# JiapengWu/TeMP

Hardware: AMD Instinct MI355X
Metric: edges/sec (fwd+bwd) RGCN+GRU seq_len=15 (higher is better)
Workload: dtype f32

## Files before the change

### temp_amd/csrc/common.hpp

```cpp
#pragma once
#include <hip/hip_runtime.h>
#include <stdint.h>
#include <stddef.h>
#include "temp_amd.h"

#define TEMP_WAVE 64

namespace temp {

typedef float f32x4 __attribute__((ext_vector_type(4)));
typedef float f32x16 __attribute__((ext_vector_type(16)));

__device__ __forceinline__ float4 ld4(const float* p) { return *reinterpret_cast<const float4*>(p); }
__device__ __forceinline__ void st4(float* p, float4 v) { *reinterpret_cast<float4*>(p) = v; }
__device__ __forceinline__ float4 ld4_nt(const float* p) {
  const f32x4 v = __builtin_nontemporal_load(reinterpret_cast<const f32x4*>(p));
  return make_float4(v[0], v[1], v[2], v[3]);
}
__device__ __forceinline__ void st4_nt(float* p, float4 v) {
  f32x4 x = {v.x, v.y, v.z, v.w};
  __builtin_nontemporal_store(x, reinterpret_cast<f32x4*>(p));
}
__device__ __forceinline__ float4 zero4() { return make_float4(0.f, 0.f, 0.f, 0.f); }
__device__ __forceinline__ float4 add4(float4 a, float4 b) { return make_float4(a.x + b.x, a.y + b.y, a.z + b.z, a.w + b.w); }
// ... 54 lines not shown
  r.end = c_hi;
  r.stride = bpx * per_block;
  return r;
}

struct DropSpec { float p; float inv_keep; unsigned long long seed; };
inline DropSpec drop_spec(const TempDropout* d) {
  DropSpec s{0.f, 1.f, 0ull};
  if (d && d->p > 0.f) { s.p = d->p; s.inv_keep = 1.f / (1.f - d->p); s.seed = d->seed; }
  return s;
}
__device__ __forceinline__ float drop_scale(const DropSpec& d, unsigned row, unsigned col) {
  unsigned long long x = d.seed ^ (((unsigned long long)row << 32) | col);
  x ^= x >> 33; x *= 0xff51afd7ed558ccdULL; x ^= x >> 33; x *= 0xc4ceb9fe1a85ec53ULL; x ^= x >> 33;
  const float u = (float)(x >> 40) * (1.0f / 16777216.0f);
  return u < d.p ? 0.f : d.inv_keep;
}
__device__ __forceinline__ float4 drop4(const DropSpec& d, unsigned row, unsigned col, float4 v) {
  return make_float4(v.x * drop_scale(d, row, col), v.y * drop_scale(d, row, col + 1), v.z * drop_scale(d, row, col + 2),
                     v.w * drop_scale(d, row, col + 3));
}

int option(int key);
void hx_count();

inline int ceil_div(long long a, long long b) { return (int)((a + b - 1) / b); }
inline size_t align_up(size_t x, size_t a) { return (x + a - 1) / a * a; }

enum KernelId {
  K_RGCN_AGG_FWD = 0, K_RGCN_AGG_DX, K_RGCN_DW, K_FIXUP, K_GEMM_LOOP_FWD, K_GEMM_LOOP_DX, K_GEMM_TN, K_REDUCE_SLICES, K_COLSUM,
  K_RELU_BWD, K_GRU_FWD, K_GRU_BWD_GATES, K_GEMM_GRU_DX, K_GEMM_GRU_DPREV, K_GATHER_ROWS, K_SCATTER_ADD, K_DECAY_GRAD, K_COPY,
  K_GEMM_ISO, K_GEMM_GRU_GI, K_GEMM_LINEAR, K_GATHER_CE, K_SA_ATTN_FWD, K_SA_ATTN_BWD, K_GRU_CHAIN_FWD, K_GRU_CHAIN_BWD,
  K_GRU_CHAIN_PACK, K_BX_PACK, K_GEMM_TN_BX8, K_GEMM_TN_BX, K_GRU_WGRAD, K_SEGMENT_SUM, K_KEYS, K_GATED_QUERY, K_GATHER_CE_MIX,
  K_PAIR_MSG, K_PAIR_GATHER_FWD, K_PAIR_FIX_EPI, K_PAIR_GATHER_BWD, K_PAIR_DTABLE, K_PAIR_DW, K_COUNT
};
int trace_open(int kernel_id, hipStream_t st);
void trace_close(int slot, hipStream_t st);
#define TEMP_LAUNCH(KID, kernel, grid, block, shmem, st, ...)            \
  do {                                                                   \
    const int _slot = ::temp::trace_open((KID), (st));                   \
    hipLaunchKernelGGL(kernel, grid, block, shmem, st, __VA_ARGS__);     \
    ::temp::trace_close(_slot, (st));                                    \
  } while (0)

inline int launch_status() {
  hipError_t e = hipGetLastError();
  return e == hipSuccess ? TEMP_OK : TEMP_E_LAUNCH;
}

struct EpiAddBiasAct;

int gemm_add_bias_act(int kid, int M, int N, int K, const float* A, int lda, const int32_t* a_idx,
                      const float* B, int ldb, int trans_b,
                      const float* addend, int ld_add, const int32_t* row_mask, const float* bias, int act,
                      float* out, int ldo, hipStream_t st, const DropSpec* drop = nullptr);

int gemm_bias_multi(int kid, int count, const int* Ms, int N, int K, const float* const* As, const int32_t* const* a_idxs , int lda,
                    const float* const* Bs, int ldb,
                    const float* const* biases, float* const* outs, int ldo, hipStream_t st,
                    const unsigned* const* a_keys = nullptr );

int mask_rows(int n, int d, const float* src, float* dst, const DropSpec& drop, hipStream_t st);

size_t gemm_tn_workspace(int M, int Ka, int Nb);
bool gemm_tn_can_fuse_bias(int Nb);
int gemm_tn(int M, int Ka, int Nb, const float* A, int lda, const float* B, int ldb,
            float* out, int ldo, void* ws, size_t ws_bytes, hipStream_t st, float* bias_out = nullptr);
// ... 21 lines not shown
```

### temp_amd/csrc/gemm_kernels.hip

```cpp
#include "common.hpp"
#include <type_traits>
#include <mutex>
#include <atomic>
#include <cstdlib>
#include "gemm_wres.hpp"
#include "gemm_tn_bx.hpp"

namespace temp {

struct EpiAddBiasAct {
  const float* addend; int ld_add; const int32_t* row_mask; const float* bias; int act; float* out; int ldo;
  struct RowCtx { int add; };
  __device__ __forceinline__ RowCtx row_ctx(int row) const {
    RowCtx c;
    c.add = !addend ? 0 : (row_mask ? row_mask[row] : 1);
    return c;
  }
  __device__ __forceinline__ float4 pre4(const RowCtx& c, int row, int col) const {
    float4 a = zero4();
    if (addend) {
      const float4 v = ld4(addend + (size_t)row * ld_add + col);
      a = c.add > 0 ? v : zero4();
    }
    if (bias) a = add4(a, ld4(bias + col));
// ... 1022 lines not shown
  g_options[TEMP_OPT_GEMM_STREAM] = 0; g_options[TEMP_OPT_GRU_STREAM] = 0; g_options[TEMP_OPT_RGCN_TILE] = 1; g_options[TEMP_OPT_DEBUG] = 0; g_options[TEMP_OPT_OVERLAP] = 1; g_options[TEMP_OPT_GEMM_RESIDENT] = 1;
  g_options[TEMP_OPT_MFMA_F16X2] = 1;
  g_options[TEMP_OPT_RGCN_PAIR] = 1;
  const char* e;
  if ((e = getenv("TEMP_MFMA")) && e[0] == 'f' && e[1] == '3') g_options[TEMP_OPT_MFMA_BF16X3] = 0;
  if ((e = getenv("TEMP_MFMA")) && e[0] == 'b') g_options[TEMP_OPT_MFMA_F16X2] = 0;
  if ((e = getenv("TEMP_TN_SPLIT")) && e[0] == '0') g_options[TEMP_OPT_TN_SPLIT] = 0;
  if ((e = getenv("TEMP_RGCN_SCALAR")) && e[0] == '0') g_options[TEMP_OPT_RGCN_SCALAR] = 0;
  if ((e = getenv("TEMP_GEMM_STREAM")) && e[0] == '1') g_options[TEMP_OPT_GEMM_STREAM] = 1;
  if ((e = getenv("TEMP_GRU_STREAM")) && e[0] == '1') g_options[TEMP_OPT_GRU_STREAM] = 1;
  if ((e = getenv("TEMP_RGCN_TILE")) && e[0] >= '0' && e[0] <= '9') g_options[TEMP_OPT_RGCN_TILE] = atoi(e);
  if ((e = getenv("TEMP_OVERLAP")) && e[0] == '0') g_options[TEMP_OPT_OVERLAP] = 0;
  if ((e = getenv("TEMP_GEMM_RESIDENT")) && e[0] == '0') g_options[TEMP_OPT_GEMM_RESIDENT] = 0;
  if ((e = getenv("TEMP_DEBUG"))) g_options[TEMP_OPT_DEBUG] = atoi(e);
  if ((e = getenv("TEMP_RGCN_PAIR")) && e[0] >= '0' && e[0] <= '9') g_options[TEMP_OPT_RGCN_PAIR] = atoi(e);
  return true;
}();
int option(int key) { return (key >= 0 && key < TEMP_OPT_COUNT) ? g_options[key].load(std::memory_order_relaxed) : -1; }
static std::atomic<long long> g_hx_launches{0};
void hx_count() { g_hx_launches.fetch_add(1, std::memory_order_relaxed); }
long long hx_launches() { return g_hx_launches.load(std::memory_order_relaxed); }
}

extern "C" {

const char* temp_trace_kernel_name(int id) {
  static const char* names[] = {"k_rgcn_agg<fwd>", "k_rgcn_agg<dx>", "k_rgcn_dw", "k_fixup", "k_gemm_panel<loop_fwd>",
                                "k_gemm_panel<loop_dx>", "k_gemm_tn", "k_reduce_slices", "k_colsum_part", "k_relu_bwd", "k_gru_fwd",
                                "k_gru_bwd_gates", "k_gemm_panel<gru_dx>", "k_gemm_panel<gru_dprev>", "k_gather_rows",
                                "k_scatter_add_rows", "k_decay_grad", "k_copy", "k_gemm_panel<isolated>", "k_gemm_panel<gru_gi>",
                                "k_gemm_panel<linear>", "k_gather_ce", "k_sa_attn_fwd", "k_sa_attn_bwd", "k_gru_chain_fwd", "k_gru_chain_bwd",
                                "k_gru_chain_pack", "k_bx_pack", "k_gemm_tn_bx8", "k_gemm_tn_bx", "k_gru_wgrad", "k_segment_sum_rows", "k_absmax_keys",
                                "k_gated_query", "k_gather_ce_mix", "k_pair_msg", "k_pair_gather<fwd>", "k_pair_fix_epi", "k_pair_gather<bwd>",
                                "k_pair_dtable", "k_pair_dw"};
  static_assert(sizeof(names) / sizeof(names[0]) == K_COUNT, "one name per KernelId");
  return (id >= 0 && id < K_COUNT) ? names[id] : "?";
}

int temp_abi_version(void) { return TEMP_ABI_VERSION; }

int temp_set_option(int key, int value) {
  if (key < 0 || key >= TEMP_OPT_COUNT) return -1;
  return temp::g_options[key].exchange(value, std::memory_order_relaxed);
}
int temp_get_option(int key) { return temp::option(key); }
long long temp_scratch_refused(void) { return temp::bx_scratch_refused(); }
long long temp_f16_launches(void) { return temp::hx_launches(); }

const char* temp_error_string(int code) {
  switch (code) {
    case TEMP_OK: return "ok";
    case TEMP_E_BADARG: return "bad argument (NULL, negative or inconsistent)";
    case TEMP_E_UNSUPPORTED: return "shape not supported by the gfx950 kernels";
    case TEMP_E_WORKSPACE: return "workspace missing or too small";
    case TEMP_E_LAUNCH: return "HIP launch failure";
    default: return "unknown error";
  }
}

int temp_rgcn_isolated_fwd(int n, int d, const float* e, const float* loop_w, const float* bias, int act, float* out, const TempDropout* drop,
                           void* stream) {
  if (n < 0 || d <= 0 || !loop_w || (n > 0 && (!e || !out))) return TEMP_E_BADARG;
  if (d % 4) return TEMP_E_UNSUPPORTED;
  const DropSpec ds = drop_spec(drop);
  return gemm_add_bias_act(K_GEMM_ISO, n, d, d, e, d, nullptr, loop_w, d, 0, e, d, nullptr, bias, act, out, d, (hipStream_t)stream, &ds);
}

// ... 650 lines not shown
```

### temp_amd/csrc/rgcn_kernels.hip

```cpp
#include <stdlib.h>
#include <atomic>
#include <mutex>
#include "common.hpp"
#include "side_stream.hpp"

namespace temp {

enum { MODE_FWD = 0, MODE_DX = 1 };

template <int S, int MODE>
__device__ __forceinline__ void block_mac(float4& acc, const float4 x, const float4* w, const float c) {
  if (S == 1) {
    acc.x = fmaf(c * x.x, w[0].x, acc.x);
    acc.y = fmaf(c * x.y, w[0].y, acc.y);
    acc.z = fmaf(c * x.z, w[0].z, acc.z);
    acc.w = fmaf(c * x.w, w[0].w, acc.w);
  } else if (S == 2) {
    const float x0 = c * x.x, x1 = c * x.y, x2 = c * x.z, x3 = c * x.w;
    if (MODE == MODE_FWD) {
      acc.x = fmaf(x0, w[0].x, fmaf(x1, w[0].z, acc.x));
      acc.y = fmaf(x0, w[0].y, fmaf(x1, w[0].w, acc.y));
      acc.z = fmaf(x2, w[1].x, fmaf(x3, w[1].z, acc.z));
      acc.w = fmaf(x2, w[1].y, fmaf(x3, w[1].w, acc.w));
    } else {
// ... 834 lines not shown
      };
      int e = 0;
      for (; e + 8 <= cnt; e += 8) {
        float4 x[8];
#pragma unroll
        for (int u = 0; u < 8; ++u) x[u] = row(e + u);
#pragma unroll
        for (int u = 0; u < 8; ++u) add(e + u, x[u]);
      }
      for (; e + 2 <= cnt; e += 2) {
        const float4 x0 = row(e), x1 = row(e + 1);
        add(e, x0);
        add(e + 1, x1);
      }
      if (e < cnt) add(e, row(e));
    }
  }
  return acc;
}

__device__ __forceinline__ float4 pair_epilogue(float4 v, int node, int f, int D, const int32_t* __restrict__ ids, const float* __restrict__ t_loop,
                                                const float* __restrict__ bias, int act, const DropSpec& drop) {
  float4 lm = ld4(t_loop + (size_t)ids[node] * D + f);
  if (drop.p > 0.f) lm = drop4(drop, (unsigned)node, (unsigned)f, lm);
  v = add4(v, lm);
  if (bias) v = add4(v, ld4(bias + f));
  if (act == TEMP_ACT_RELU) v = make_float4(fmaxf(v.x, 0.f), fmaxf(v.y, 0.f), fmaxf(v.z, 0.f), fmaxf(v.w, 0.f));
  return v;
}

__global__ void __launch_bounds__(256) k_pair_gather_fwd(TempEdgeView v, const int32_t* __restrict__ fwd_row, const float* __restrict__ M,
                                                         const float* __restrict__ nnorm, int D, const int32_t* __restrict__ ids,
                                                         const float* __restrict__ t_loop, const float* __restrict__ bias, int act, DropSpec drop,
                                                         float* __restrict__ out, float* __restrict__ partial) {
  const int lane = threadIdx.x & 63;
  const int wave = __builtin_amdgcn_readfirstlane(threadIdx.x >> 6), wpb = blockDim.x >> 6;
  const int f = lane << 2;
  const bool active = lane < (D >> 2);
  ItemRange it = xcd_chunks(v.n_chunks, v.n_edges, v.chunk_beg, wpb);
  for (int c = it.beg + wave; c < it.end; c += it.stride) {
    const int seg = __builtin_amdgcn_readfirstlane(v.chunk_seg[c]), beg = __builtin_amdgcn_readfirstlane(v.chunk_beg[c]);
    const int end = __builtin_amdgcn_readfirstlane(v.chunk_end[c]), slot = __builtin_amdgcn_readfirstlane(v.chunk_slot[c]);
    float4 acc = pair_rows_sum<false>(fwd_row, beg, end, M, D, nullptr, lane, active);
    if (!active) continue;
    const float nn = nnorm[seg];
    acc = scale4(acc, nn * nn);
    if (slot < 0) st4(out + (size_t)seg * D + f, pair_epilogue(acc, seg, f, D, ids, t_loop, bias, act, drop));
    else st4(partial + (size_t)slot * D + f, acc);
  }
}

__global__ void __launch_bounds__(256) k_pair_fix_epi(int n_fix, const int32_t* __restrict__ fix_seg, const int32_t* __restrict__ fix_slot,
                                                      const int32_t* __restrict__ fix_cnt, const float* __restrict__ partial, int n_nodes,
                                                      const int32_t* __restrict__ in_deg, int D, const int32_t* __restrict__ ids,
                                                      const float* __restrict__ t_loop, const float* __restrict__ bias, int act, DropSpec drop,
                                                      float* __restrict__ out) {
  const int lane = threadIdx.x & 63, wpb = blockDim.x >> 6;
  const int gw = blockIdx.x * wpb + (threadIdx.x >> 6), waves = gridDim.x * wpb;
  const int f = lane << 2;
  if (f >= D) return;
  for (int i = gw; i < n_fix; i += waves) {
    const int seg = fix_seg[i];
    st4(out + (size_t)seg * D + f, pair_epilogue(fixup_walk(partial + (size_t)fix_slot[i] * D + f, 0, fix_cnt[i], D), seg, f, D, ids, t_loop, bias, act, drop));
  }
  for (int node = gw; node < n_nodes; node += waves)
    if (in_deg[node] <= 0) st4(out + (size_t)node * D + f, pair_epilogue(zero4(), node, f, D, ids, t_loop, bias, act, drop));
}

__global__ void __launch_bounds__(256) k_pair_gather_bwd(TempEdgeView v, const float* __restrict__ dz, const float* __restrict__ nnorm, int D,
                                                         float* __restrict__ G, float* __restrict__ partial) {
  const int lane = threadIdx.x & 63;
  const int wave = __builtin_amdgcn_readfirstlane(threadIdx.x >> 6), wpb = blockDim.x >> 6;
  const int f = lane << 2;
  const bool active = lane < (D >> 2);
  for (int c = blockIdx.x * wpb + wave; c < v.n_chunks; c += gridDim.x * wpb) {
    const int seg = __builtin_amdgcn_readfirstlane(v.chunk_seg[c]), beg = __builtin_amdgcn_readfirstlane(v.chunk_beg[c]);
    const int end = __builtin_amdgcn_readfirstlane(v.chunk_end[c]), slot = __builtin_amdgcn_readfirstlane(v.chunk_slot[c]);
    const float4 acc = pair_rows_sum<true>(v.a, beg, end, dz, D, nnorm, lane, active);
    if (active) st4((slot < 0 ? G + (size_t)seg * D : partial + (size_t)slot * D) + f, acc);
  }
}

template <int S>
__global__ void __launch_bounds__(64) k_pair_dtable(int n_table, int n_rel_rows, int D, const float* __restrict__ G, const float* __restrict__ W,
                                                    float* __restrict__ d_table) {
  const int D4 = D >> 2;
  const int i = blockIdx.x * blockDim.x + threadIdx.x;
  if (i >= n_table * D4) return;
  const int e = i / D4, f = (i - e * D4) << 2;
  float4 acc = zero4();
#pragma unroll 4
  for (int r = 0; r < n_rel_rows; ++r) {
    const float* wr = W + (size_t)r * (D * S) + f * S;
    float4 w[S];
#pragma unroll
    for (int j = 0; j < S; ++j) w[j] = ld4(wr + 4 * j);
    block_mac<S, MODE_DX>(acc, ld4(G + ((size_t)r * n_table + e) * D + f), w, 1.f);
  }
  st4(d_table + (size_t)e * D + f, acc);
}

template <int S>
__global__ void __launch_bounds__(1024) k_pair_dw(int n_table, int D, const float* __restrict__ table, const float* __restrict__ G,
                                                  float* __restrict__ dW) {
  __shared__ float4 share[16][64];
  const int lane = threadIdx.x & 63, wave = __builtin_amdgcn_readfirstlane(threadIdx.x >> 6);
  const int r = blockIdx.x, f = lane << 2;
  const bool active = f < D;
  const int per = (n_table + 15) >> 4;
  const int e0 = min(n_table, wave * per), e1 = min(n_table, e0 + per);
  float4 acc[S];
#pragma unroll
  for (int j = 0; j < S; ++j) acc[j] = zero4();
  if (active) {
    const float* g = G + (size_t)r * n_table * D + f;
#pragma unroll 4
    for (int e = e0; e < e1; ++e) {
      const float4 xx = ld4(table + (size_t)e * D + f), gg = ld4(g + (size_t)e * D);
      if (S == 1) {
        acc[0].x = fmaf(xx.x, gg.x, acc[0].x);
        acc[0].y = fmaf(xx.y, gg.y, acc[0].y);
        acc[0].z = fmaf(xx.z, gg.z, acc[0].z);
        acc[0].w = fmaf(xx.w, gg.w, acc[0].w);
      } else if (S == 2) {
        acc[0].x = fmaf(xx.x, gg.x, acc[0].x);
        acc[0].y = fmaf(xx.x, gg.y, acc[0].y);
        acc[0].z = fmaf(xx.y, gg.x, acc[0].z);
        acc[0].w = fmaf(xx.y, gg.y, acc[0].w);
        acc[1].x = fmaf(xx.z, gg.z, acc[1].x);
        acc[1].y = fmaf(xx.z, gg.w, acc[1].y);
        acc[1].z = fmaf(xx.w, gg.z, acc[1].z);
        acc[1].w = fmaf(xx.w, gg.w, acc[1].w);
      } else {
        acc[0] = fma4(xx.x, gg, acc[0]);
        acc[1] = fma4(xx.y, gg, acc[1]);
        acc[2] = fma4(xx.z, gg, acc[2]);
        acc[3] = fma4(xx.w, gg, acc[3]);
      }
    }
  }
#pragma unroll
  for (int j = 0; j < S; ++j) {
    share[wave][lane] = acc[j];
    __syncthreads();
    if (wave == 0 && active) {
      float4 t = share[0][lane];
#pragma unroll
      for (int u = 1; u < 16; ++u) t = add4(t, share[u][lane]);
      st4(dW + (size_t)r * (D * S) + f * S + 4 * j, t);
    }
    __syncthreads();
  }
}

__global__ void __launch_bounds__(256) k_expand_chunk_seg(int n_chunks, const int32_t* __restrict__ chunk_seg, const int32_t* __restrict__ chunk_beg,
                                                          const int32_t* __restrict__ chunk_end, int n_pos, int32_t* __restrict__ seg_of) {
  const int lane = threadIdx.x & 63, wpb = blockDim.x >> 6;
  for (int c = blockIdx.x * wpb + (threadIdx.x >> 6); c < n_chunks; c += gridDim.x * wpb) {
    const int seg = chunk_seg[c], beg = max(0, chunk_beg[c]), end = min(n_pos, chunk_end[c]);
    for (int p = beg + lane; p < end; p += 64) seg_of[p] = seg;
  }
}

static bool pair_view_ok(const TempGraph* g, const TempPairView* pv, int n_table, int n_rel_rows) {
  if (!g || !pv || pv->n_table != n_table || pv->n_rel_rows != n_rel_rows) return false;
  const TempEdgeView& v = pv->by_pair;
  if (v.n_seg != n_rel_rows * n_table + 1 || v.n_chunks < 0 || v.n_partial < 0 || v.n_fix < 0) return false;
  if ((v.n_edges > 0 && !v.a) || !v.chunk_seg || !v.chunk_beg || !v.chunk_end || !v.chunk_slot) return false;
  if (v.n_fix > 0 && (!v.fix_seg || !v.fix_slot || !v.fix_cnt)) return false;
  return g->by_dst.n_edges == 0 || pv->fwd_row != nullptr;
}

struct PairFwdWs { float *partial, *t_loop, *M; size_t total; };
static PairFwdWs carve_pair_fwd(const TempGraph* g, const TempPairView* pv, int d_out, char* base) {
  PairFwdWs w;
  size_t off = 0;
  auto take = [&](size_t bytes) { char* p = base ? base + off : nullptr; off += align_up(bytes, 256); return p; };
  w.partial = (float*)take((size_t)g->by_dst.n_partial * d_out * sizeof(float));
  w.t_loop = (float*)take((size_t)pv->n_table * d_out * sizeof(float));
  w.M = (float*)take((size_t)pv->n_rel_rows * pv->n_table * d_out * sizeof(float));
  w.total = off + 256;
  return w;
}

struct PairBwdWs {
  float *dz, *dzm, *G, *part, *seg_dz;
  void *ss, *tn, *cs;
  size_t ss_bytes, tn_bytes, cs_bytes, total;
};
static PairBwdWs carve_pair_bwd(const TempGraph* g, const TempPairView* pv, int d_in, int d_out, char* base) {
  PairBwdWs w;
  size_t off = 0;
  auto take = [&](size_t bytes) { char* p = base ? base + off : nullptr; off += align_up(bytes, 256); return p; };
  w.dz = (float*)take((size_t)g->n_nodes * d_out * sizeof(float));
  w.dzm = (float*)take((size_t)g->n_nodes * d_out * sizeof(float));
  w.G = (float*)take((size_t)pv->by_pair.n_seg * d_out * sizeof(float));
  w.part = (float*)take(partial_bytes(pv->by_pair.n_partial, d_out));
  w.seg_dz = (float*)take((size_t)pv->n_table * d_out * sizeof(float));
  w.ss_bytes = segment_sum_rows_workspace(pv->n_table, g->n_nodes, d_out);
  w.ss = take(w.ss_bytes);
  w.tn_bytes = gemm_tn_workspace(pv->n_table, d_in, d_out);
  w.tn = take(w.tn_bytes);
  w.cs_bytes = colsum_workspace(g->n_nodes, d_out);
  w.cs = take(w.cs_bytes);
  w.total = off + 256;
  return w;
}

struct TableBwdWs {
  float *dz, *dzm, *d_h, *part_dx, *part_dw, *seg_dz;
  void *tn, *cs;
  size_t tn_bytes, cs_bytes, total;
};
static TableBwdWs carve_table_bwd(const TempGraph* g, int n_table, int d_in, int d_out, int num_bases, char* base) {
  TableBwdWs w;
  size_t off = 0;
  auto take = [&](size_t bytes) { char* p = base ? base + off : nullptr; off += align_up(bytes, 256); return p; };
  const size_t wrow = (size_t)num_bases * (d_in / num_bases) * (d_out / num_bases);
  w.dz = (float*)take((size_t)g->n_nodes * d_out * sizeof(float));
  w.dzm = (float*)take((size_t)g->n_nodes * d_out * sizeof(float));
  w.d_h = (float*)take((size_t)g->n_nodes * d_in * sizeof(float));
  w.part_dx = (float*)take(partial_bytes(g->by_src.n_partial, d_in));
  w.part_dw = (float*)take(partial_bytes(g->by_rel.n_partial, wrow));
  w.seg_dz = (float*)take((size_t)n_table * d_out * sizeof(float));
  w.tn_bytes = gemm_tn_workspace(n_table, d_in, d_out);
  w.tn = take(w.tn_bytes);
  w.cs_bytes = colsum_workspace(g->n_nodes, d_out);
  w.cs = take(w.cs_bytes);
  w.total = off + 256;
  return w;
}
// ... 122 lines not shown
  int S = 0;
  return fast_shape(d_in, d_out, num_bases, &S) ? 1 : 0;
}

size_t temp_rgcn_pair_fwd_workspace(const TempGraph* g, const TempPairView* pv, int d_out) {
  if (!g || !pv || d_out <= 0 || pv->n_table < 0 || pv->n_rel_rows < 0) return 0;
  return carve_pair_fwd(g, pv, d_out, nullptr).total;
}

int temp_rgcn_pair_fwd(const TempGraph* g, const TempPairView* pv, const float* table, const int32_t* ids, int n_table, int d_in, int d_out,
                       int num_bases, int n_rel_rows, const float* weight, const float* loop_w, const float* bias, int act, float* out,
                       void* workspace, size_t workspace_bytes, const TempDropout* drop, void* stream) {
  if (!g || !pv || !table || !weight || !loop_w || !out || n_table <= 0 || d_in <= 0 || d_out <= 0 || num_bases <= 0 || n_rel_rows <= 0) return TEMP_E_BADARG;
  int S = 0;
  if (!fast_shape(d_in, d_out, num_bases, &S)) return TEMP_E_UNSUPPORTED;
  if ((long long)n_rel_rows * n_table >= (1LL << 31) / d_out) return TEMP_E_UNSUPPORTED;
  if (g->n_nodes < 0 || !view_ok(g->by_dst) || !pair_view_ok(g, pv, n_table, n_rel_rows) || (g->n_nodes > 0 && (!g->nnorm || !g->in_deg || !ids))) return TEMP_E_BADARG;
  if (act != TEMP_ACT_NONE && act != TEMP_ACT_RELU) return TEMP_E_BADARG;
  if (!workspace || workspace_bytes < temp_rgcn_pair_fwd_workspace(g, pv, d_out)) return TEMP_E_WORKSPACE;
  if (g->n_nodes == 0) return TEMP_OK;
  hipStream_t st = (hipStream_t)stream;
  const PairFwdWs w = carve_pair_fwd(g, pv, d_out, (char*)workspace);
  const int D = d_in, P = n_rel_rows * n_table;
  int grid = ceil_div((long long)P * (D / 4), 256);
  if (grid > 8192) grid = 8192;
  if (S == 1) TEMP_LAUNCH(K_PAIR_MSG, k_pair_msg<1>, dim3(grid), dim3(256), 0, st, P, n_table, D, table, weight, w.M);
  else if (S == 2) TEMP_LAUNCH(K_PAIR_MSG, k_pair_msg<2>, dim3(grid), dim3(256), 0, st, P, n_table, D, table, weight, w.M);
  else TEMP_LAUNCH(K_PAIR_MSG, k_pair_msg<4>, dim3(grid), dim3(256), 0, st, P, n_table, D, table, weight, w.M);
  int rc = gemm_add_bias_act(K_GEMM_ISO, n_table, d_out, d_in, table, d_in, nullptr, loop_w, d_out, 0, nullptr, 0, nullptr, nullptr, TEMP_ACT_NONE,
                             w.t_loop, d_out, st);
  if (rc) return rc;
  const DropSpec ds = drop_spec(drop);
  const TempEdgeView& v = g->by_dst;
  if (v.n_chunks > 0) {
    grid = (v.n_chunks + 3) / 4;
    grid = grid < 8 ? 8 : (grid > 4096 ? 4096 : (grid + 7) / 8 * 8);
    TEMP_LAUNCH(K_PAIR_GATHER_FWD, k_pair_gather_fwd, dim3(grid), dim3(256), 0, st, v, pv->fwd_row, w.M, g->nnorm, D, ids, w.t_loop, bias, act, ds, out,
                w.partial);
  }
  const int items = v.n_fix > (g->n_nodes + 7) / 8 ? v.n_fix : (g->n_nodes + 7) / 8;
  grid = (items + 3) / 4;
  if (grid > 4096) grid = 4096;
  TEMP_LAUNCH(K_PAIR_FIX_EPI, k_pair_fix_epi, dim3(grid), dim3(256), 0, st, v.n_fix, v.fix_seg, v.fix_slot, v.fix_cnt, w.partial, g->n_nodes, g->in_deg, D,
              ids, w.t_loop, bias, act, ds, out);
  g_pair_launches.fetch_add(1, std::memory_order_relaxed);
  return launch_status();
}

size_t temp_rgcn_pair_bwd_workspace(const TempGraph* g, const TempPairView* pv, int d_in, int d_out, int num_bases) {
  if (!g || !pv || num_bases <= 0 || d_in <= 0 || d_out <= 0 || pv->n_table < 0 || pv->by_pair.n_seg < 0) return 0;
  return carve_pair_bwd(g, pv, d_in, d_out, nullptr).total;
}

int temp_rgcn_pair_bwd(const TempGraph* g, const TempPairView* pv, const float* table, const int32_t* ids, const int32_t* inv_ptr,
                       const int32_t* inv_order, int n_table, const float* out, const float* d_out_grad, int d_in, int d_out, int num_bases,
                       int n_rel_rows, const float* weight, const float* loop_w, int has_bias, int act, float* d_table, float* d_weight,
                       float* d_loop_w, float* d_bias, void* workspace, size_t workspace_bytes, const TempDropout* drop, void* stream) {
  if (!g || !pv || !table || !d_out_grad || !weight || !loop_w || !d_table || !d_weight || !d_loop_w || !inv_ptr) return TEMP_E_BADARG;
  if (n_table <= 0 || d_in <= 0 || d_out <= 0 || num_bases <= 0 || n_rel_rows <= 0) return TEMP_E_BADARG;
  int S = 0;
  if (!fast_shape(d_in, d_out, num_bases, &S)) return TEMP_E_UNSUPPORTED;
  if ((long long)n_rel_rows * n_table >= (1LL << 31) / d_out) return TEMP_E_UNSUPPORTED;
  if (act == TEMP_ACT_RELU && !out) return TEMP_E_BADARG;
  if (act != TEMP_ACT_NONE && act != TEMP_ACT_RELU) return TEMP_E_BADARG;
  if (has_bias && !d_bias) return TEMP_E_BADARG;
  if (g->n_nodes < 0 || !pair_view_ok(g, pv, n_table, n_rel_rows) || (g->n_nodes > 0 && (!g->nnorm || !ids || !inv_order))) return TEMP_E_BADARG;
  if (!workspace || workspace_bytes < temp_rgcn_pair_bwd_workspace(g, pv, d_in, d_out, num_bases)) return TEMP_E_WORKSPACE;
  hipStream_t st = (hipStream_t)stream;
  const size_t wrow = (size_t)d_in * S;
  if (g->n_nodes == 0) {
    if (hipMemsetAsync(d_table, 0, (size_t)n_table * d_in * sizeof(float), st) != hipSuccess) return TEMP_E_LAUNCH;
    if (hipMemsetAsync(d_weight, 0, (size_t)n_rel_rows * wrow * sizeof(float), st) != hipSuccess) return TEMP_E_LAUNCH;
    if (hipMemsetAsync(d_loop_w, 0, (size_t)d_in * d_out * sizeof(float), st) != hipSuccess) return TEMP_E_LAUNCH;
    if (has_bias && hipMemsetAsync(d_bias, 0, (size_t)d_out * sizeof(float), st) != hipSuccess) return TEMP_E_LAUNCH;
    return TEMP_OK;
  }
  const PairBwdWs w = carve_pair_bwd(g, pv, d_in, d_out, (char*)workspace);
  const int D = d_in;
  const float* dz = d_out_grad;
  int rc;
  if (act == TEMP_ACT_RELU) {
    rc = relu_bwd((size_t)g->n_nodes * d_out, out, d_out_grad, w.dz, st);
    if (rc) return rc;
    dz = w.dz;
  }
  const TempEdgeView& v = pv->by_pair;
  int grid = (v.n_chunks + 3) / 4;
  grid = grid < 1 ? 1 : (grid > 4096 ? 4096 : grid);
  TEMP_LAUNCH(K_PAIR_GATHER_BWD, k_pair_gather_bwd, dim3(grid), dim3(256), 0, st, v, dz, g->nnorm, D, w.G, w.part);
  launch_fixup(v, w.part, D, w.G, st);
  grid = ceil_div((long long)n_table * (D / 4), 64);
  if (S == 1) TEMP_LAUNCH(K_PAIR_DTABLE, k_pair_dtable<1>, dim3(grid), dim3(64), 0, st, n_table, n_rel_rows, D, w.G, weight, d_table);
  else if (S == 2) TEMP_LAUNCH(K_PAIR_DTABLE, k_pair_dtable<2>, dim3(grid), dim3(64), 0, st, n_table, n_rel_rows, D, w.G, weight, d_table);
  else TEMP_LAUNCH(K_PAIR_DTABLE, k_pair_dtable<4>, dim3(grid), dim3(64), 0, st, n_table, n_rel_rows, D, w.G, weight, d_table);
  if (S == 1) TEMP_LAUNCH(K_PAIR_DW, k_pair_dw<1>, dim3(n_rel_rows), dim3(1024), 0, st, n_table, D, table, w.G, d_weight);
  else if (S == 2) TEMP_LAUNCH(K_PAIR_DW, k_pair_dw<2>, dim3(n_rel_rows), dim3(1024), 0, st, n_table, D, table, w.G, d_weight);
  else TEMP_LAUNCH(K_PAIR_DW, k_pair_dw<4>, dim3(n_rel_rows), dim3(1024), 0, st, n_table, D, table, w.G, d_weight);
  const DropSpec ds = drop_spec(drop);
  const float* dzm = dz;
  if (ds.p > 0.f) {
    rc = mask_rows(g->n_nodes, d_out, dz, w.dzm, ds, st);
    if (rc) return rc;
    dzm = w.dzm;
  }
  rc = segment_sum_rows(n_table, d_out, inv_ptr, inv_order, dzm, nullptr, w.seg_dz, st, g->n_nodes, w.ss, w.ss_bytes);
  if (rc) return rc;
  rc = gemm_add_bias_act(K_GEMM_LOOP_DX, n_table, d_in, d_out, w.seg_dz, d_out, nullptr, loop_w, d_out, 1, d_table, d_in, nullptr, nullptr,
                         TEMP_ACT_NONE, d_table, d_in, st);
  if (rc) return rc;
  rc = gemm_tn(n_table, d_in, d_out, table, d_in, w.seg_dz, d_out, d_loop_w, d_out, w.tn, w.tn_bytes, st);
  if (rc) return rc;
  if (has_bias) {
    rc = colsum(g->n_nodes, d_out, dz, d_out, d_bias, w.cs, w.cs_bytes, st);
    if (rc) return rc;
  }
  g_pair_launches.fetch_add(1, std::memory_order_relaxed);
  return launch_status();
}

size_t temp_rgcn_fwd_workspace(const TempGraph* g, int d_out) {
  if (!g) return 0;
  return partial_bytes(g->by_dst.n_partial, d_out) + 256;
}

int temp_rgcn_fwd(const TempGraph* g, const float* h, const int32_t* h_ids, int d_in, int d_out, int num_bases, int n_rel_rows,
                  const float* weight, const float* loop_w, const float* bias, int act, float* out, void* workspace,
                  size_t workspace_bytes, const TempDropout* drop, void* stream) {
  if (!g || !h || !weight || !loop_w || !out || d_in <= 0 || d_out <= 0 || num_bases <= 0 || n_rel_rows <= 0) return TEMP_E_BADARG;
  if (d_in % num_bases || d_out % num_bases || d_in % 4 || d_out % 4) return TEMP_E_UNSUPPORTED;
  if (g->n_nodes < 0 || !view_ok(g->by_dst) || (g->n_nodes > 0 && (!g->nnorm || !g->in_deg))) return TEMP_E_BADARG;
  if (act != TEMP_ACT_NONE && act != TEMP_ACT_RELU) return TEMP_E_BADARG;
  if (workspace_bytes < temp_rgcn_fwd_workspace(g, d_out) || (!workspace && g->by_dst.n_partial > 0)) return TEMP_E_WORKSPACE;
  if (g->n_nodes == 0) return TEMP_OK;
  hipStream_t st = (hipStream_t)stream;
  float* partial = (float*)workspace;
  int rc = run_agg(MODE_FWD, g->by_dst, members_of(g), h, d_in, h_ids, weight, n_rel_rows, g->nnorm, d_in, d_out, num_bases, out, partial, st);
  if (rc) return rc;
  const DropSpec ds = drop_spec(drop);
  return gemm_add_bias_act(K_GEMM_LOOP_FWD, g->n_nodes, d_out, d_in, h, d_in, h_ids, loop_w, d_out, 0, out, d_out, g->in_deg, bias, act, out, d_out, st, &ds);
}

struct BwdWs {
  float* dz;
  float* dzm;
  float* part_dx;
  float* part_dw;
  void* tn;
  size_t tn_bytes;
// ... 156 lines not shown
```

Measured before the change: 900.6 million.

## Fuse pair dtable and dW into one tiled tail kernel and overlap loop-grad work on a side stream

The separate k_pair_dtable and k_pair_dw kernels become one k_pair_tail kernel. Each block tiles 8 table rows and splits relation rows across waves, so every G tile is read once for both the d_table and the dW accumulation. Per-block dW partials are then summed with reduce_slices. The self-loop backward chain (mask, segment_sum, loop dx GEMM, gemm_tn, colsum) is forked onto a side stream to overlap with the gather backward. Its dx result goes to a workspace buffer that the tail kernel adds into d_table. In the forward pass, writing zero-in-degree nodes moves from fix_epi into the gather kernel, and fix_epi is skipped when there are no fixups. The costs are extra workspace, a reduction pass, and cross-stream synchronization.

```diff
diff --git a/temp_amd/csrc/common.hpp b/temp_amd/csrc/common.hpp
--- a/temp_amd/csrc/common.hpp
+++ b/temp_amd/csrc/common.hpp
@@ -110,7 +110,7 @@
   K_RELU_BWD, K_GRU_FWD, K_GRU_BWD_GATES, K_GEMM_GRU_DX, K_GEMM_GRU_DPREV, K_GATHER_ROWS, K_SCATTER_ADD, K_DECAY_GRAD, K_COPY,
   K_GEMM_ISO, K_GEMM_GRU_GI, K_GEMM_LINEAR, K_GATHER_CE, K_SA_ATTN_FWD, K_SA_ATTN_BWD, K_GRU_CHAIN_FWD, K_GRU_CHAIN_BWD,
   K_GRU_CHAIN_PACK, K_BX_PACK, K_GEMM_TN_BX8, K_GEMM_TN_BX, K_GRU_WGRAD, K_SEGMENT_SUM, K_KEYS, K_GATED_QUERY, K_GATHER_CE_MIX,
-  K_PAIR_MSG, K_PAIR_GATHER_FWD, K_PAIR_FIX_EPI, K_PAIR_GATHER_BWD, K_PAIR_DTABLE, K_PAIR_DW, K_COUNT
+  K_PAIR_MSG, K_PAIR_GATHER_FWD, K_PAIR_FIX_EPI, K_PAIR_GATHER_BWD, K_PAIR_TAIL, K_COUNT
 };
 int trace_open(int kernel_id, hipStream_t st);
 void trace_close(int slot, hipStream_t st);
diff --git a/temp_amd/csrc/gemm_kernels.hip b/temp_amd/csrc/gemm_kernels.hip
--- a/temp_amd/csrc/gemm_kernels.hip
+++ b/temp_amd/csrc/gemm_kernels.hip
@@ -1078,7 +1078,7 @@
                                 "k_gemm_panel<linear>", "k_gather_ce", "k_sa_attn_fwd", "k_sa_attn_bwd", "k_gru_chain_fwd", "k_gru_chain_bwd",
                                 "k_gru_chain_pack", "k_bx_pack", "k_gemm_tn_bx8", "k_gemm_tn_bx", "k_gru_wgrad", "k_segment_sum_rows", "k_absmax_keys",
                                 "k_gated_query", "k_gather_ce_mix", "k_pair_msg", "k_pair_gather<fwd>", "k_pair_fix_epi", "k_pair_gather<bwd>",
-                                "k_pair_dtable", "k_pair_dw"};
+                                "k_pair_tail"};
   static_assert(sizeof(names) / sizeof(names[0]) == K_COUNT, "one name per KernelId");
   return (id >= 0 && id < K_COUNT) ? names[id] : "?";
 }
diff --git a/temp_amd/csrc/rgcn_kernels.hip b/temp_amd/csrc/rgcn_kernels.hip
--- a/temp_amd/csrc/rgcn_kernels.hip
+++ b/temp_amd/csrc/rgcn_kernels.hip
@@ -890,7 +890,8 @@
 __global__ void __launch_bounds__(256) k_pair_gather_fwd(TempEdgeView v, const int32_t* __restrict__ fwd_row, const float* __restrict__ M,
                                                          const float* __restrict__ nnorm, int D, const int32_t* __restrict__ ids,
                                                          const float* __restrict__ t_loop, const float* __restrict__ bias, int act, DropSpec drop,
-                                                         float* __restrict__ out, float* __restrict__ partial) {
+                                                         float* __restrict__ out, float* __restrict__ partial, int n_nodes,
+                                                         const int32_t* __restrict__ in_deg) {
   const int lane = threadIdx.x & 63;
   const int wave = __builtin_amdgcn_readfirstlane(threadIdx.x >> 6), wpb = blockDim.x >> 6;
   const int f = lane << 2;
@@ -906,13 +907,21 @@
     if (slot < 0) st4(out + (size_t)seg * D + f, pair_epilogue(acc, seg, f, D, ids, t_loop, bias, act, drop));
     else st4(partial + (size_t)slot * D + f, acc);
   }
+  const int gw = blockIdx.x * wpb + wave, waves = gridDim.x * wpb;
+  for (int n0 = gw * 64; n0 < n_nodes; n0 += waves * 64) {
+    unsigned long long m = __ballot(n0 + lane < n_nodes && in_deg[n0 + lane] <= 0);
+    while (m) {
+      const int node = n0 + __ffsll((long long)m) - 1;
+      m &= m - 1;
+      if (active) st4(out + (size_t)node * D + f, pair_epilogue(zero4(), node, f, D, ids, t_loop, bias, act, drop));
+    }
+  }
 }
 
 __global__ void __launch_bounds__(256) k_pair_fix_epi(int n_fix, const int32_t* __restrict__ fix_seg, const int32_t* __restrict__ fix_slot,
-                                                      const int32_t* __restrict__ fix_cnt, const float* __restrict__ partial, int n_nodes,
-                                                      const int32_t* __restrict__ in_deg, int D, const int32_t* __restrict__ ids,
-                                                      const float* __restrict__ t_loop, const float* __restrict__ bias, int act, DropSpec drop,
-                                                      float* __restrict__ out) {
+                                                      const int32_t* __restrict__ fix_cnt, const float* __restrict__ partial, int D,
+                                                      const int32_t* __restrict__ ids, const float* __restrict__ t_loop,
+                                                      const float* __restrict__ bias, int act, DropSpec drop, float* __restrict__ out) {
   const int lane = threadIdx.x & 63, wpb = blockDim.x >> 6;
   const int gw = blockIdx.x * wpb + (threadIdx.x >> 6), waves = gridDim.x * wpb;
   const int f = lane << 2;
@@ -921,8 +930,6 @@
     const int seg = fix_seg[i];
     st4(out + (size_t)seg * D + f, pair_epilogue(fixup_walk(partial + (size_t)fix_slot[i] * D + f, 0, fix_cnt[i], D), seg, f, D, ids, t_loop, bias, act, drop));
   }
-  for (int node = gw; node < n_nodes; node += waves)
-    if (in_deg[node] <= 0) st4(out + (size_t)node * D + f, pair_epilogue(zero4(), node, f, D, ids, t_loop, bias, act, drop));
 }
 
 __global__ void __launch_bounds__(256) k_pair_gather_bwd(TempEdgeView v, const float* __restrict__ dz, const float* __restrict__ nnorm, int D,
@@ -940,75 +947,96 @@
 }
 
 template <int S>
-__global__ void __launch_bounds__(64) k_pair_dtable(int n_table, int n_rel_rows, int D, const float* __restrict__ G, const float* __restrict__ W,
-                                                    float* __restrict__ d_table) {
-  const int D4 = D >> 2;
-  const int i = blockIdx.x * blockDim.x + threadIdx.x;
-  if (i >= n_table * D4) return;
-  const int e = i / D4, f = (i - e * D4) << 2;
-  float4 acc = zero4();
-#pragma unroll 4
-  for (int r = 0; r < n_rel_rows; ++r) {
-    const float* wr = W + (size_t)r * (D * S) + f * S;
-    float4 w[S];
-#pragma unroll
-    for (int j = 0; j < S; ++j) w[j] = ld4(wr + 4 * j);
-    block_mac<S, MODE_DX>(acc, ld4(G + ((size_t)r * n_table + e) * D + f), w, 1.f);
-  }
-  st4(d_table + (size_t)e * D + f, acc);
-}
-
+__device__ __forceinline__ void block_outer(float4* acc, const float4 xx, const float4 gg) {
+  if (S == 1) {
+    acc[0].x = fmaf(xx.x, gg.x, acc[0].x);
+    acc[0].y = fmaf(xx.y, gg.y, acc[0].y);
+    acc[0].z = fmaf(xx.z, gg.z, acc[0].z);
+    acc[0].w = fmaf(xx.w, gg.w, acc[0].w);
+  } else if (S == 2) {
+    acc[0].x = fmaf(xx.x, gg.x, acc[0].x);
+    acc[0].y = fmaf(xx.x, gg.y, acc[0].y);
+    acc[0].z = fmaf(xx.y, gg.x, acc[0].z);
+    acc[0].w = fmaf(xx.y, gg.y, acc[0].w);
+    acc[1].x = fmaf(xx.z, gg.z, acc[1].x);
+    acc[1].y = fmaf(xx.z, gg.w, acc[1].y);
+    acc[1].z = fmaf(xx.w, gg.z, acc[1].z);
+    acc[1].w = fmaf(xx.w, gg.w, acc[1].w);
+  } else {
+    acc[0] = fma4(xx.x, gg, acc[0]);
+    acc[1] = fma4(xx.y, gg, acc[1]);
+    acc[2] = fma4(xx.z, gg, acc[2]);
+    acc[3] = fma4(xx.w, gg, acc[3]);
+  }
+}
+
+#define PT_TE 8
+#define PT_WAVES 8
+#define PT_MAX_BLOCKS 128
 template <int S>
-__global__ void __launch_bounds__(1024) k_pair_dw(int n_table, int D, const float* __restrict__ table, const float* __restrict__ G,
-                                                  float* __restrict__ dW) {
-  __shared__ float4 share[16][64];
+__global__ void __launch_bounds__(PT_WAVES * 64) k_pair_tail(int n_table, int n_rel_rows, int D, int tiles_per_block, const float* __restrict__ G,
+                                                             const float* __restrict__ W, const float* __restrict__ table,
+                                                             const float* __restrict__ add, float* __restrict__ d_table,
+                                                             float* __restrict__ dw_part) {
+  __shared__ float4 share[PT_WAVES][PT_TE][64];
   const int lane = threadIdx.x & 63, wave = __builtin_amdgcn_readfirstlane(threadIdx.x >> 6);
-  const int r = blockIdx.x, f = lane << 2;
+  const int f = lane << 2;
   const bool active = f < D;
-  const int per = (n_table + 15) >> 4;
-  const int e0 = min(n_table, wave * per), e1 = min(n_table, e0 + per);
-  float4 acc[S];
-#pragma unroll
-  for (int j = 0; j < S; ++j) acc[j] = zero4();
-  if (active) {
-    const float* g = G + (size_t)r * n_table * D + f;
-#pragma unroll 4
-    for (int e = e0; e < e1; ++e) {
-      const float4 xx = ld4(table + (size_t)e * D + f), gg = ld4(g + (size_t)e * D);
-      if (S == 1) {
-        acc[0].x = fmaf(xx.x, gg.x, acc[0].x);
-        acc[0].y = fmaf(xx.y, gg.y, acc[0].y);
-        acc[0].z = fmaf(xx.z, gg.z, acc[0].z);
-        acc[0].w = fmaf(xx.w, gg.w, acc[0].w);
-      } else if (S == 2) {
-        acc[0].x = fmaf(xx.x, gg.x, acc[0].x);
-        acc[0].y = fmaf(xx.x, gg.y, acc[0].y);
-        acc[0].z = fmaf(xx.y, gg.x, acc[0].z);
-        acc[0].w = fmaf(xx.y, gg.y, acc[0].w);
-        acc[1].x = fmaf(xx.z, gg.z, acc[1].x);
-        acc[1].y = fmaf(xx.z, gg.w, acc[1].y);
-        acc[1].z = fmaf(xx.w, gg.z, acc[1].z);
-        acc[1].w = fmaf(xx.w, gg.w, acc[1].w);
-      } else {
-        acc[0] = fma4(xx.x, gg, acc[0]);
-        acc[1] = fma4(xx.y, gg, acc[1]);
-        acc[2] = fma4(xx.z, gg, acc[2]);
-        acc[3] = fma4(xx.w, gg, acc[3]);
-      }
-    }
-  }
-#pragma unroll
-  for (int j = 0; j < S; ++j) {
-    share[wave][lane] = acc[j];
+  const int per = (n_rel_rows + PT_WAVES - 1) / PT_WAVES;
+  const int r0 = min(n_rel_rows, wave * per), r1 = min(n_rel_rows, r0 + per);
+  const int n_act = (n_rel_rows + per - 1) / per;
+  const size_t wrow = (size_t)D * S;
+  float* my_part = dw_part + (size_t)blockIdx.x * n_rel_rows * wrow;
+  for (int t = 0; t < tiles_per_block; ++t) {
+    const int e0 = (blockIdx.x * tiles_per_block + t) * PT_TE;
+    if (e0 >= n_table) break;
+    float4 acc[PT_TE], x[PT_TE];
+#pragma unroll
+    for (int u = 0; u < PT_TE; ++u) acc[u] = zero4();
+    if (active) {
+#pragma unroll
+      for (int u = 0; u < PT_TE; ++u) x[u] = e0 + u < n_table ? ld4(table + (size_t)(e0 + u) * D + f) : zero4();
+      for (int r = r0; r < r1; ++r) {
+        const float* wr = W + (size_t)r * wrow + f * S;
+        const float* gr = G + ((size_t)r * n_table + e0) * D + f;
+        float4 w[S], dw[S], g[PT_TE];
+#pragma unroll
+        for (int u = 0; u < PT_TE; ++u) g[u] = e0 + u < n_table ? ld4(gr + (size_t)u * D) : zero4();
+#pragma unroll
+        for (int j = 0; j < S; ++j) { w[j] = ld4(wr + 4 * j); dw[j] = zero4(); }
+#pragma unroll
+        for (int u = 0; u < PT_TE; ++u) {
+          block_mac<S, MODE_DX>(acc[u], g[u], w, 1.f);
+          block_outer<S>(dw, x[u], g[u]);
+        }
+        float* p = my_part + (size_t)r * wrow + f * S;
+#pragma unroll
+        for (int j = 0; j < S; ++j) st4(p + 4 * j, t > 0 ? add4(ld4(p + 4 * j), dw[j]) : dw[j]);
+      }
+    }
+    if (wave < n_act) {
+#pragma unroll
+      for (int u = 0; u < PT_TE; ++u) share[wave][u][lane] = acc[u];
+    }
     __syncthreads();
-    if (wave == 0 && active) {
-      float4 t = share[0][lane];
-#pragma unroll
-      for (int u = 1; u < 16; ++u) t = add4(t, share[u][lane]);
-      st4(dW + (size_t)r * (D * S) + f * S + 4 * j, t);
+    const int e = e0 + wave;
+    if (active && e < n_table) {
+      float4 s = share[0][wave][lane];
+      for (int q = 1; q < n_act; ++q) s = add4(s, share[q][wave][lane]);
+      if (add) s = add4(s, ld4(add + (size_t)e * D + f));
+      st4(d_table + (size_t)e * D + f, s);
     }
     __syncthreads();
   }
+}
+static_assert(PT_WAVES == PT_TE, "k_pair_tail: one wave per table row of the tile in the d_table reduction");
+struct PairTailGrid { int blocks, tiles_per_block; };
+static PairTailGrid pair_tail_grid(int n_table) {
+  const int tiles = ceil_div(n_table > 0 ? n_table : 1, PT_TE);
+  PairTailGrid t;
+  t.tiles_per_block = ceil_div(tiles, PT_MAX_BLOCKS);
+  t.blocks = ceil_div(tiles, t.tiles_per_block);
+  return t;
 }
 
 __global__ void __launch_bounds__(256) k_expand_chunk_seg(int n_chunks, const int32_t* __restrict__ chunk_seg, const int32_t* __restrict__ chunk_beg,
@@ -1042,11 +1070,11 @@
 }
 
 struct PairBwdWs {
-  float *dz, *dzm, *G, *part, *seg_dz;
+  float *dz, *dzm, *G, *part, *seg_dz, *loop_dt, *dw_part;
   void *ss, *tn, *cs;
   size_t ss_bytes, tn_bytes, cs_bytes, total;
 };
-static PairBwdWs carve_pair_bwd(const TempGraph* g, const TempPairView* pv, int d_in, int d_out, char* base) {
+static PairBwdWs carve_pair_bwd(const TempGraph* g, const TempPairView* pv, int d_in, int d_out, int S, char* base) {
   PairBwdWs w;
   size_t off = 0;
   auto take = [&](size_t bytes) { char* p = base ? base + off : nullptr; off += align_up(bytes, 256); return p; };
@@ -1055,6 +1083,8 @@
   w.G = (float*)take((size_t)pv->by_pair.n_seg * d_out * sizeof(float));
   w.part = (float*)take(partial_bytes(pv->by_pair.n_partial, d_out));
   w.seg_dz = (float*)take((size_t)pv->n_table * d_out * sizeof(float));
+  w.loop_dt = (float*)take((size_t)pv->n_table * d_in * sizeof(float));
+  w.dw_part = (float*)take((size_t)pair_tail_grid(pv->n_table).blocks * pv->n_rel_rows * d_in * S * sizeof(float));
   w.ss_bytes = segment_sum_rows_workspace(pv->n_table, g->n_nodes, d_out);
   w.ss = take(w.ss_bytes);
   w.tn_bytes = gemm_tn_workspace(pv->n_table, d_in, d_out);
@@ -1243,24 +1273,26 @@
   if (rc) return rc;
   const DropSpec ds = drop_spec(drop);
   const TempEdgeView& v = g->by_dst;
-  if (v.n_chunks > 0) {
-    grid = (v.n_chunks + 3) / 4;
-    grid = grid < 8 ? 8 : (grid > 4096 ? 4096 : (grid + 7) / 8 * 8);
-    TEMP_LAUNCH(K_PAIR_GATHER_FWD, k_pair_gather_fwd, dim3(grid), dim3(256), 0, st, v, pv->fwd_row, w.M, g->nnorm, D, ids, w.t_loop, bias, act, ds, out,
-                w.partial);
-  }
-  const int items = v.n_fix > (g->n_nodes + 7) / 8 ? v.n_fix : (g->n_nodes + 7) / 8;
+  const int items = v.n_chunks > (g->n_nodes + 63) / 64 ? v.n_chunks : (g->n_nodes + 63) / 64;
   grid = (items + 3) / 4;
-  if (grid > 4096) grid = 4096;
-  TEMP_LAUNCH(K_PAIR_FIX_EPI, k_pair_fix_epi, dim3(grid), dim3(256), 0, st, v.n_fix, v.fix_seg, v.fix_slot, v.fix_cnt, w.partial, g->n_nodes, g->in_deg, D,
-              ids, w.t_loop, bias, act, ds, out);
+  grid = grid < 8 ? 8 : (grid > 4096 ? 4096 : (grid + 7) / 8 * 8);
+  TEMP_LAUNCH(K_PAIR_GATHER_FWD, k_pair_gather_fwd, dim3(grid), dim3(256), 0, st, v, pv->fwd_row, w.M, g->nnorm, D, ids, w.t_loop, bias, act, ds, out,
+              w.partial, g->n_nodes, g->in_deg);
+  if (v.n_fix > 0) {
+    grid = (v.n_fix + 3) / 4;
+    if (grid > 4096) grid = 4096;
+    TEMP_LAUNCH(K_PAIR_FIX_EPI, k_pair_fix_epi, dim3(grid), dim3(256), 0, st, v.n_fix, v.fix_seg, v.fix_slot, v.fix_cnt, w.partial, D, ids, w.t_loop,
+                bias, act, ds, out);
+  }
   g_pair_launches.fetch_add(1, std::memory_order_relaxed);
   return launch_status();
 }
 
 size_t temp_rgcn_pair_bwd_workspace(const TempGraph* g, const TempPairView* pv, int d_in, int d_out, int num_bases) {
-  if (!g || !pv || num_bases <= 0 || d_in <= 0 || d_out <= 0 || pv->n_table < 0 || pv->by_pair.n_seg < 0) return 0;
-  return carve_pair_bwd(g, pv, d_in, d_out, nullptr).total;
+  if (!g || !pv || num_bases <= 0 || d_in <= 0 || d_out <= 0 || pv->n_table < 0 || pv->n_rel_rows < 0 || pv->by_pair.n_seg < 0) return 0;
+  int S = 0;
+  if (!fast_shape(d_in, d_out, num_bases, &S)) S = 4;
+  return carve_pair_bwd(g, pv, d_in, d_out, S, nullptr).total;
 }
 
 int temp_rgcn_pair_bwd(const TempGraph* g, const TempPairView* pv, const float* table, const int32_t* ids, const int32_t* inv_ptr,
@@ -1286,7 +1318,7 @@
     if (has_bias && hipMemsetAsync(d_bias, 0, (size_t)d_out * sizeof(float), st) != hipSuccess) return TEMP_E_LAUNCH;
     return TEMP_OK;
   }
-  const PairBwdWs w = carve_pair_bwd(g, pv, d_in, d_out, (char*)workspace);
+  const PairBwdWs w = carve_pair_bwd(g, pv, d_in, d_out, S, (char*)workspace);
   const int D = d_in;
   const float* dz = d_out_grad;
   int rc;
@@ -1295,36 +1327,36 @@
     if (rc) return rc;
     dz = w.dz;
   }
+  SideScope side(st);
+  const bool beside = !(option(TEMP_OPT_DEBUG) & 0x800000) && side_fork(side);
+  hipStream_t sl = beside ? side.ss->s : st;
+  const DropSpec ds = drop_spec(drop);
+  const float* dzm = dz;
+  rc = TEMP_OK;
+  if (ds.p > 0.f) {
+    rc = mask_rows(g->n_nodes, d_out, dz, w.dzm, ds, sl);
+    dzm = w.dzm;
+  }
+  if (!rc) rc = segment_sum_rows(n_table, d_out, inv_ptr, inv_order, dzm, nullptr, w.seg_dz, sl, g->n_nodes, w.ss, w.ss_bytes);
+  if (!rc) rc = gemm_add_bias_act(K_GEMM_LOOP_DX, n_table, d_in, d_out, w.seg_dz, d_out, nullptr, loop_w, d_out, 1, nullptr, 0, nullptr, nullptr,
+                                  TEMP_ACT_NONE, w.loop_dt, d_in, sl);
+  if (!rc) rc = gemm_tn(n_table, d_in, d_out, table, d_in, w.seg_dz, d_out, d_loop_w, d_out, w.tn, w.tn_bytes, sl);
+  if (!rc && has_bias) rc = colsum(g->n_nodes, d_out, dz, d_out, d_bias, w.cs, w.cs_bytes, sl);
+  if (beside && !side_done(side) && !rc) rc = TEMP_E_LAUNCH;
+  if (rc) return rc;
   const TempEdgeView& v = pv->by_pair;
   int grid = (v.n_chunks + 3) / 4;
   grid = grid < 1 ? 1 : (grid > 4096 ? 4096 : grid);
   TEMP_LAUNCH(K_PAIR_GATHER_BWD, k_pair_gather_bwd, dim3(grid), dim3(256), 0, st, v, dz, g->nnorm, D, w.G, w.part);
   launch_fixup(v, w.part, D, w.G, st);
-  grid = ceil_div((long long)n_table * (D / 4), 64);
-  if (S == 1) TEMP_LAUNCH(K_PAIR_DTABLE, k_pair_dtable<1>, dim3(grid), dim3(64), 0, st, n_table, n_rel_rows, D, w.G, weight, d_table);
-  else if (S == 2) TEMP_LAUNCH(K_PAIR_DTABLE, k_pair_dtable<2>, dim3(grid), dim3(64), 0, st, n_table, n_rel_rows, D, w.G, weight, d_table);
-  else TEMP_LAUNCH(K_PAIR_DTABLE, k_pair_dtable<4>, dim3(grid), dim3(64), 0, st, n_table, n_rel_rows, D, w.G, weight, d_table);
-  if (S == 1) TEMP_LAUNCH(K_PAIR_DW, k_pair_dw<1>, dim3(n_rel_rows), dim3(1024), 0, st, n_table, D, table, w.G, d_weight);
-  else if (S == 2) TEMP_LAUNCH(K_PAIR_DW, k_pair_dw<2>, dim3(n_rel_rows), dim3(1024), 0, st, n_table, D, table, w.G, d_weight);
-  else TEMP_LAUNCH(K_PAIR_DW, k_pair_dw<4>, dim3(n_rel_rows), dim3(1024), 0, st, n_table, D, table, w.G, d_weight);
-  const DropSpec ds = drop_spec(drop);
-  const float* dzm = dz;
-  if (ds.p > 0.f) {
-    rc = mask_rows(g->n_nodes, d_out, dz, w.dzm, ds, st);
-    if (rc) return rc;
-    dzm = w.dzm;
-  }
-  rc = segment_sum_rows(n_table, d_out, inv_ptr, inv_order, dzm, nullptr, w.seg_dz, st, g->n_nodes, w.ss, w.ss_bytes);
+  rc = side.join();
   if (rc) return rc;
-  rc = gemm_add_bias_act(K_GEMM_LOOP_DX, n_table, d_in, d_out, w.seg_dz, d_out, nullptr, loop_w, d_out, 1, d_table, d_in, nullptr, nullptr,
-                         TEMP_ACT_NONE, d_table, d_in, st);
-  if (rc) return rc;
-  rc = gemm_tn(n_table, d_in, d_out, table, d_in, w.seg_dz, d_out, d_loop_w, d_out, w.tn, w.tn_bytes, st);
-  if (rc) return rc;
-  if (has_bias) {
-    rc = colsum(g->n_nodes, d_out, dz, d_out, d_bias, w.cs, w.cs_bytes, st);
-    if (rc) return rc;
-  }
+  const PairTailGrid tg = pair_tail_grid(n_table);
+  float* dwp = tg.blocks > 1 ? w.dw_part : d_weight;
+  if (S == 1) TEMP_LAUNCH(K_PAIR_TAIL, k_pair_tail<1>, dim3(tg.blocks), dim3(PT_WAVES * 64), 0, st, n_table, n_rel_rows, D, tg.tiles_per_block, w.G, weight, table, w.loop_dt, d_table, dwp);
+  else if (S == 2) TEMP_LAUNCH(K_PAIR_TAIL, k_pair_tail<2>, dim3(tg.blocks), dim3(PT_WAVES * 64), 0, st, n_table, n_rel_rows, D, tg.tiles_per_block, w.G, weight, table, w.loop_dt, d_table, dwp);
+  else TEMP_LAUNCH(K_PAIR_TAIL, k_pair_tail<4>, dim3(tg.blocks), dim3(PT_WAVES * 64), 0, st, n_table, n_rel_rows, D, tg.tiles_per_block, w.G, weight, table, w.loop_dt, d_table, dwp);
+  if (tg.blocks > 1) reduce_slices(tg.blocks, (size_t)n_rel_rows * wrow, (int)wrow, w.dw_part, d_weight, (int)wrow, st);
   g_pair_launches.fetch_add(1, std::memory_order_relaxed);
   return launch_status();
 }
```

Result: faster. 914.4 million (median of 6 runs) (+1.5%).
